# Audio-WestlakeU/NBSS

Measured on AMD Instinct MI355X. Metric: utterances/sec (4 s, 6ch, 129 freqs) SpatialNet bf16 train at 1/2/4/8 MI355X, higher is better.
Workload: dtype bf16; 1 GPU; SpatialNet-small 6ch->2spk, 4-s 8-kHz utterances (32000 samples), n_fft 256/hop 128 (F=129, T=251), 8 layers, full train step (STFT..Adam), bf16 stream + fp32 master/stats, 32 utterances per GPU per step; batch_per_gpu=32, global_batch=32, parallelism=dp1

## Files before the change

nbss_amd/csrc/tconvffn_s.hip:

```cpp
#include "side.h"
#include "launch.h"
#include "layout.h"
#include "prof.h"
#include "fold.h"
#include "foldk.h"

#define TS_H 96
#define TS_FFN 192
#define TS_G 8
#define TS_CG 24
#define TS_RS 200
#define TS_PAD 4
#define TS_ONE 0x3F80u
#define TS_WL_FR 56

typedef float f32x16 __attribute__((ext_vector_type(16)));
typedef Frag<bf16_t> FragH;

NBSS_DEV f32x16 mma32(const FragH& a, const FragH& b, f32x16 c) {
#ifdef NBSS_EMU
    return hipemu::mfma_32x32x16_bf16(a.v, b.v, c);
#else
    return __builtin_amdgcn_mfma_f32_32x32x16_bf16(a.v, b.v, c, 0, 0, 0);
#endif
// ... 774 lines not shown
                        pa.d[i] = pack2bf(a3[2 * i], a3[2 * i + 1]) & vm;
                        const float v0 = bf_lo(pa.d[i]), v1 = bf_hi(pa.d[i]);
                        s1 += v0 + v1;
                        s2 += v0 * v0 + v1 * v1;
                    }
                    p6_store(orow(t, 2, 6), pa);
                }
        }
        s1 = wave_sum64(s1);
        s2 = wave_sum64(s2);
        if (L.lane == 0) {
            red[(gl * 2 + th) * 2] = s1;
            red[(gl * 2 + th) * 2 + 1] = s2;
        }
    }
    load_wfrags<5>(wb, W.C2T, g, L.lane);
    PHASE(6);
    lds_barrier();
    PHASE(7);
    const float gmean = (red[gl * 4] + red[gl * 4 + 2]) / cnt;
    const float grstd = rsqrtf(fmaxf((red[gl * 4 + 1] + red[gl * 4 + 3]) / cnt - gmean * gmean, 0.f) + 1e-5f);
#pragma unroll 2
    for (int s = s_beg; s < s_end; ++s) {
        const int t = 32 * s + L.n;
        const bool tv = t < T_;
        const uint32_t vm = lane_mask(tv);
        bf16_t* r = orow(t, 2, 6);
        P6 pa, pn, ph;
        p6_load(r, pa);
        float a3[12], hv[12];
        p6_unpack(pa, a3);
#pragma unroll
        for (int q = 0; q < 12; ++q) a3[q] = (a3[q] - gmean) * grstd;
        p6_pack(a3, vm, pn);
        p6_unpack(pn, a3);
#pragma unroll
        for (int q = 0; q < 12; ++q) hv[q] = silu_f(a3[q] * gw[q] + gb[q]);
        p6_pack(hv, vm, ph);
        p6_store(Bc + (size_t)t * TB_RS, pn);
        p6_store(r, ph);
    }
    run_gstore(ops.h4, 2, 6);
    PHASE(8);
    lds_barrier();
    PHASE(9);
#pragma unroll 1
    TB_BLOCKS(true) {
        FragH b[TB_SB][5];
        P6 p5[TB_SB];
#pragma unroll
        for (int k = 0; k < TB_SB; ++k)
            if (s0 + k < s_end) {
                const int t = 32 * (s0 + k) + L.n;
                conv_bfrags3(L, rowp(t - 1, 2, 6), rowp(t, 2, 6), rowp(t + 1, 2, 6), b[k]);
                const int pi = s0 + k - s_beg;
#pragma unroll
                for (int i = 0; i < 6; ++i) {
                    const uint32_t lo = pi == 0 ? park0.d[i] : park1.d[i], hi = pi == 2 ? park2.d[i] : park3.d[i];
                    p5[k].d[i] = pi < 2 ? lo : hi;
                }
            }
#pragma unroll
        for (int k = 0; k < TB_SB; ++k)
            if (s0 + k < s_end) {
                const int t = 32 * (s0 + k) + L.n;
                const bool tv = t < T_;
                const uint32_t vm = lane_mask(tv);
                const f32x16 a5 = conv_mma(wc, b[k]);
                float hv[12], dv[12], d5[12];
                p6_unpack(p5[k], d5);
#pragma unroll
                for (int r = 0; r < 12; ++r) {
                    silu_dsilu(a5[r], hv[r], dv[r]);
                    dv[r] *= d5[r];
                }
                P6 ph, pd;
                p6_pack(hv, vm, ph);
                p6_pack(dv, vm, pd);
                p6_store(orow(t, 1, 7), pd);
                p6_gstore(ops.h5 + gbase + (size_t)t * TS_CG, ph, tv, true);
            }
    }
    run_gstore(ops.da5, 1, 7);
    load_wfrags<5>(wc, W.C3T, g, L.lane);
    PHASE(10);
    lds_barrier();
    PHASE(11);
    fetch_cross(1, 7);
    {
        float sa = 0.f, sb = 0.f, dgw[12], dgb[12];
#pragma unroll
        for (int r = 0; r < 12; ++r) dgw[r] = dgb[r] = 0.f;
#pragma unroll 1
        TB_BLOCKS(false) {
            FragH b[TB_SB][5];
#pragma unroll
            for (int k = 0; k < TB_SB; ++k)
                if (s0 + k < s_end) {
                    const int t = 32 * (s0 + k) + L.n;
                    conv_bfrags3(L, rowx(t - 1, 1, 7), rowp(t, 1, 7), rowx(t + 1, 1, 7), b[k]);
                }
#pragma unroll
            for (int k = 0; k < TB_SB; ++k)
                if (s0 + k < s_end) {
                    const int t = 32 * (s0 + k) + L.n;
                    const uint32_t vm = lane_mask(t < T_);
                    const f32x16 dh4 = conv_mma(wc, b[k]);
                    P6 pn, pd;
                    p6_load(Bc + (size_t)t * TB_RS, pn);
                    float ah[12], dn[12];
                    p6_unpack(pn, ah);
#pragma unroll
                    for (int r = 0; r < 12; ++r) dn[r] = dh4[r] * dsilu_only(ah[r] * gw[r] + gb[r]);
                    p6_pack(dn, vm, pd);
                    p6_unpack(pd, dn);
#pragma unroll
                    for (int r = 0; r < 12; ++r) {
                        dgw[r] += dn[r] * ah[r];
                        dgb[r] += dn[r];
                        sa += gw[r] * dn[r];
                        sb += gw[r] * dn[r] * ah[r];
                    }
                    p6_store(orow(t, 2, 6), pd);
                }
        }
        sa = wave_sum64(sa);
        sb = wave_sum64(sb);
        if (L.lane == 0) {
            red[(gl * 2 + th) * 2] = sa;
            red[(gl * 2 + th) * 2 + 1] = sb;
        }
#pragma unroll
        for (int r = 0; r < 12; ++r) {
            const float a = half_sum32(dgw[r]), bq = half_sum32(dgb[r]);
            if (L.n == 0) {
                const int ch = gl * TS_CG + (r & 3) + 8 * (r >> 2) + 4 * L.h;
                gnp[(th * 2 + 0) * 96 + ch] = a;
                gnp[(th * 2 + 1) * 96 + ch] = bq;
            }
        }
        if (L.lane < 6) *reinterpret_cast<u32x2*>(Sc + (size_t)(th ? NT + 6 : 1) * TB_RS + 4 * L.lane) = (u32x2){0u, 0u};
    }
    PHASE(12);
    lds_barrier();
    PHASE(13);
    {
        const float msa = (red[gl * 4] + red[gl * 4 + 2]) / cnt, msb = (red[gl * 4 + 1] + red[gl * 4 + 3]) / cnt;
#pragma unroll 2
        for (int s = s_beg; s < s_end; ++s) {
            const int t = 32 * s + L.n;
            const bool tv = t < T_;
            const uint32_t vm = lane_mask(tv);
            bf16_t* r = orow(t, 2, 6);
            P6 pd, pn, po;
            p6_load(r, pd);
            p6_load(Bc + (size_t)t * TB_RS, pn);
            float dn[12], ah[12];
            p6_unpack(pd, dn);
            p6_unpack(pn, ah);
#pragma unroll
            for (int q = 0; q < 12; ++q) dn[q] = grstd * (gw[q] * dn[q] - msa - ah[q] * msb);
            p6_pack(dn, vm, po);
            p6_store(r, po);
        }
        run_gstore(ops.da3, 2, 6);
    }
    PHASE(14);
    lds_barrier();
    PHASE(15);
    fetch_cross(2, 6);
#pragma unroll 1
    TB_BLOCKS(false) {
        FragH b[TB_SB][5];
#pragma unroll
        for (int k = 0; k < TB_SB; ++k)
            if (s0 + k < s_end) {
                const int t = 32 * (s0 + k) + L.n;
                conv_bfrags3(L, rowx(t - 1, 2, 6), rowp(t, 2, 6), rowx(t + 1, 2, 6), b[k]);
            }
#pragma unroll
        for (int k = 0; k < TB_SB; ++k)
            if (s0 + k < s_end) {
                const int t = 32 * (s0 + k) + L.n;
                const bool tv = t < T_;
                const uint32_t vm = lane_mask(tv);
                const f32x16 dh2 = conv_mma(wb, b[k]);
                P6 pd2, po;
                p6_load(Ac + (size_t)t * TB_RS, pd2);
                float d2[12], o[12];
                p6_unpack(pd2, d2);
#pragma unroll
                for (int r = 0; r < 12; ++r) o[r] = dh2[r] * d2[r];
                p6_pack(o, vm, po);
                p6_store(orow(t, 3, 5), po);
            }
    }
    run_gstore(ops.da2, 3, 5);
    if (L.lane < 6) *reinterpret_cast<u32x2*>(Sc + (size_t)(th ? NT + 5 : 2) * TB_RS + 4 * L.lane) = (u32x2){0u, 0u};
    PHASE(16);
    lds_barrier();
    PHASE(17);
    fetch_cross(3, 5);
#pragma unroll 1
    TB_BLOCKS(false) {
        FragH b[TB_SB][5];
#pragma unroll
        for (int k = 0; k < TB_SB; ++k)
            if (s0 + k < s_end) {
                const int t = 32 * (s0 + k) + L.n;
                conv_bfrags3(L, rowx(t - 1, 3, 5), rowp(t, 3, 5), rowx(t + 1, 3, 5), b[k]);
            }
#pragma unroll
        for (int k = 0; k < TB_SB; ++k)
            if (s0 + k < s_end) {
                const int t = 32 * (s0 + k) + L.n;
                const f32x16 dh1 = conv_mma(wa, b[k]);
                float o[12];
#pragma unroll
                for (int r = 0; r < 12; ++r) o[r] = dh1[r];
                P6 po;
                p6_pack(o, 0xFFFFFFFFu, po);
                p6_store(orow(t, 4, 4), po);
            }
    }
    PHASE(18);
    lds_barrier();
    if (w < NS) {
        const int t = 32 * w + L.n;
        const bool tv = t < T_;
#pragma unroll
        for (int q = 0; q < 4; ++q) {
            P6 ph, po;
            p6_load(S + (size_t)(4 + t) * TB_RS + q * TS_CG + 4 * L.h, ph);
            float dh[12], d1[12];
            p6_unpack(ph, dh);
            p6_unpack(d1keep[q], d1);
#pragma unroll
            for (int r = 0; r < 12; ++r) dh[r] *= d1[r];
            p6_pack(dh, lane_mask(tv), po);
            p6_store(S + (size_t)(4 + t) * TB_RS + q * TS_CG + 4 * L.h, po);
        }
        wave_lds_sync();
#pragma unroll
        for (int q = 0; q < 4; ++q)
            rows_gstore<96>(ops.da1 + ((size_t)(4 * gh + q) * ntok + n0 + 32 * w) * TS_CG, S + (size_t)(4 + 32 * w) * TB_RS + q * TS_CG, 32, T_ - 32 * w);
    }
#undef TB_BLOCKS
    for (int i = tid; i < 2 * 96; i += blockDim.x) {
        const int kind = i / 96, ch = i % 96;
        part[(size_t)row * pstride + kind * TS_FFN + gh * 96 + ch] = gnp[(0 * 2 + kind) * 96 + ch] + gnp[(1 * 2 + kind) * 96 + ch];
    }
    PHASE_END();
}
PHASE_READER(nbss_phase_read_tconvffn_bwd_s)

int tconvffn_bwd_s_launch(const nbss_cfg& c, const LayerPtrs& lp, float* part, const void* packed, int layer, const void* x, const void* dy,
                          void* const* opsv, float* stats, int pstride, hipStream_t st) {
    if (c.dtype != NBSS_BF16 || c.T > 256) return NBSS_EUNSUPPORTED;
    const size_t NT = (size_t)((c.T + 31) / 32) * 32;
    const size_t a_el = NT * TB_RS > (size_t)52 * 512 ? NT * TB_RS : (size_t)52 * 512;
    const size_t lds = ((NT + TB_PAD) * TB_RS + a_el + NT * TB_RS) * sizeof(bf16_t) + (16 + 4 * 96) * sizeof(float) + 8 * TS_CG * sizeof(bf16_t) + PHASE_LDS_BYTES;
    if (lds > 160 * 1024) return NBSS_EUNSUPPORTED;
    const bf16_t* pk = (const bf16_t*)packed;
    TsBwdW W = {pk + pack_off(c, layer, K_TS_W1),  pk + pack_off(c, layer, K_TS_W2_T), pk + pack_off(c, layer, K_TS_C1),  pk + pack_off(c, layer, K_TS_C2),
                pk + pack_off(c, layer, K_TS_C3),  pk + pack_off(c, layer, K_TS_C1_T), pk + pack_off(c, layer, K_TS_C2_T), pk + pack_off(c, layer, K_TS_C3_T)};
    TsOps ops = {(bf16_t*)opsv[0], (bf16_t*)opsv[1], (bf16_t*)opsv[2], (bf16_t*)opsv[3], (bf16_t*)opsv[4], (bf16_t*)opsv[5], (bf16_t*)opsv[6], (bf16_t*)opsv[7]};
    int e = NBSS_SET_MAX_LDS(tconvffn_bwd_s_kernel, lds);
    if (e) return e;
    NBSS_LAUNCH(tconvffn_bwd_s_kernel, dim3(2 * c.B * c.F), dim3(512), lds, st, c, lp, W, (const bf16_t*)x, (const bf16_t*)dy, part, ops, stats, pstride);
    return NBSS_CHECK_LAUNCH();
}

struct TvIn {
    const bf16_t *a1, *a2, *a3;
    const float* gn;
};
struct TvW {
    const bf16_t *W2T, *C1T, *C2T, *C3T, *C3;
};
#define TV_CONVW (TS_FFN * TS_CG * 3)
#define TQ_RS 56
#define TQ_PSTRIDE (5 * TS_FFN)
#define TQ_P16 (3 * TV_CONVW)

template <int RS>
NBSS_DEV void tv_contract_t(const bf16_t* Sg, const bf16_t* Hg, int bl, int bu, int NS, int NSL, int mt, f32x4 (&acc)[5], f32x4& bsum) {
    const int lane = lane_id(), l15 = lane & 15, g4 = lane >> 4;
    const int rowoff = 8 * (g4 >> 1) + (g4 & 1) + 2 * (l15 >> 2);
    int boff[5];
#pragma unroll
    for (int j = 0; j < 5; ++j) {
        int pc = 4 * j + (l15 & 3);
        pc = pc < 18 ? pc : 17;
        const int tap = pc / 6, ch4 = pc - 6 * tap;
        boff[j] = (tap + rowoff) * RS + 4 * ch4;
    }
    const int aoff = rowoff * RS + 16 * mt + 4 * (l15 & 3);
    Frag<bf16_t> ones;
#pragma unroll
    for (int jq = 0; jq < 8; ++jq) frag_set(ones, jq, 1.0f);
#pragma unroll
    for (int j = 0; j < 5; ++j) acc[j] = F32X4_ZERO;
    bsum = F32X4_ZERO;
    for (int ks = 0; ks < NS; ++ks) {
        const int base = (ks < NSL ? bl : bu) + 32 * ks;
        Frag<bf16_t> fa, fb[5];
        frag_load_tr(fa, Sg + (size_t)base * RS + aoff, RS);
#pragma unroll
        for (int j = 0; j < 5; ++j) frag_load_tr(fb[j], Hg + (size_t)(32 * ks) * RS + boff[j], RS);
        bsum = mma(fa, ones, bsum);
#pragma unroll
        for (int j = 0; j < 5; ++j) acc[j] = mma(fa, fb[j], acc[j]);
    }
}
NBSS_DEV void tv_flush(bf16_t* __restrict__ w16, float* __restrict__ brow, int g, int mt, const f32x4 (&acc)[5], const f32x4& bsum) {
    const int lane = lane_id(), l15 = lane & 15, g4 = lane >> 4;
    const int oc0 = 16 * mt + 4 * g4;
    if (oc0 < TS_CG) {
        const int o0 = g * TS_CG + oc0;
#pragma unroll
        for (int j = 0; j < 5; ++j) {
            const int pc = 4 * j + (l15 >> 2);
            if (pc < 18) {
                const int tap = pc / 6, i = (pc - 6 * tap) * 4 + (l15 & 3);
                const u32x2 v = {pack2bf(acc[j][0], acc[j][1]), pack2bf(acc[j][2], acc[j][3])};
                *reinterpret_cast<u32x2*>(w16 + (((size_t)g * 3 + tap) * TS_CG + i) * TS_CG + oc0) = v;
            }
        }
        if (l15 == 0) {
#pragma unroll
            for (int r = 0; r < 4; ++r) brow[o0 + r] = bsum[r];
        }
    }
}

#define TV_RSL 64
static_assert(TS_H == FK_H && TS_FFN == FK_FFN && TS_CG == FK_TCG && TV_CONVW == FK_TCONVW, "foldk.h");
__global__ __launch_bounds__(256) void tconv_part_reduce1_kernel(const bf16_t* __restrict__ part16, int nrows, float* __restrict__ slices, int P16) {
    fk_p16_slices(part16, nrows, slices, P16, (int)blockIdx.x, (int)blockIdx.y, (int)gridDim.y);
}
__global__ __launch_bounds__(256) void tconv_part_reduce2_kernel(const float* __restrict__ slices, int nsl, float* __restrict__ G, long long off0, long long off1, long long off2,
                                                                 long long off3, int P16) {
    fk_tconv_final(slices, nsl, G, off0, off1, off2, off3, P16, (int)blockIdx.x);
}

__global__ __launch_bounds__(256, 2) void tconvffn_bwd_q_kernel(nbss_cfg c, LayerPtrs lp, TvW W, TvIn sv, const bf16_t* __restrict__ dy, float* __restrict__ part,
                                                                bf16_t* __restrict__ part16, bf16_t* __restrict__ op_h5, bf16_t* __restrict__ op_da1, int flip) {
    NBSS_LDS(smem);
    const int T_ = c.T, NS = (T_ + 31) >> 5, NT = NS * 32, NSL = NS >> 1, TS = 32 * NSL;
    bf16_t* S = reinterpret_cast<bf16_t*>(smem);
    bf16_t* H = S + (size_t)(NT + TB_PAD) * TQ_RS;
    const size_t h_el = (size_t)(NT + 2) * TQ_RS > (size_t)12 * 512 ? (size_t)(NT + 2) * TQ_RS : (size_t)12 * 512;
    float* red = reinterpret_cast<float*>(H + h_el);
    float* gnp = red + 8;
    bf16_t* mbox = reinterpret_cast<bf16_t*>(gnp + 4 * 48);
    bf16_t* wl = H;
    PHASE_BEGIN(mbox + 4 * TS_CG);
    const TsLane L;
    const int w = wave_id_u(), tid = threadIdx.x;
    const int row0 = blockIdx.x >> 2, gq = blockIdx.x & 3, row = flip ? (int)(gridDim.x >> 2) - 1 - row0 : row0;
    const size_t n0 = (size_t)row * T_, ntok = (size_t)c.B * c.F * T_;
    const bf16_t* dyb = dy + n0 * TS_H;

    const int gl = w >> 1, th = w & 1, g = 2 * gq + gl;
    const int s_beg = th ? NSL : 0, s_end = th ? NS : NSL, nblk = (s_end - s_beg + TB_SB - 1) / TB_SB;
    const size_t gsv = ((size_t)g * ntok + n0) * TS_CG + 4 * L.h;
    P6 pn0, pn1, pn2, pn3, pd0, pd1, pd2, pd3, ra0, ra1, ra2, ra3;
#define TV_LOADA(k, src, dst)                                                        \
    {                                                                                \
        const int t_ = 32 * (s_beg + (k)) + L.n, tc_ = t_ < T_ ? t_ : T_ - 1;        \
        if (s_beg + (k) < s_end) p6_gload((src) + gsv + (size_t)tc_ * TS_CG, dst);   \
        else                                                                         \
            for (int i_ = 0; i_ < 6; ++i_) dst.d[i_] = 0u;                           \
    }
#define TV_LOADA4(src) TV_LOADA(0, src, ra0) TV_LOADA(1, src, ra1) TV_LOADA(2, src, ra2) TV_LOADA(3, src, ra3)
    {
        u32x4 wr[3];
#pragma unroll
        for (int i = 0; i < 3; ++i) wr[i] = reinterpret_cast<const u32x4*>(W.W2T + (size_t)gq * 12 * 512)[tid + i * 256];
        u32x4 rawd[2][6];
#pragma unroll
        for (int k2 = 0; k2 < 2; ++k2) {
            const int t = 32 * (w + 4 * k2) + L.n, tc = t < T_ ? t : T_ - 1;
#pragma unroll
            for (int ks = 0; ks < 6; ++ks) rawd[k2][ks] = *reinterpret_cast<const u32x4*>(dyb + (size_t)tc * TS_H + 16 * ks + 8 * L.h);
        }
        TV_LOADA4(sv.a3)
        for (int i = tid; i < 4 * TQ_RS / 2; i += 256) reinterpret_cast<uint32_t*>(S)[i] = 0u;
        for (int i = tid; i < 5 * TQ_RS / 2; i += 256) reinterpret_cast<uint32_t*>(S + (size_t)(NT + 4) * TQ_RS)[i] = 0u;
#pragma unroll
        for (int i = 0; i < 3; ++i) reinterpret_cast<u32x4*>(wl)[tid + i * 256] = wr[i];
        PHASE(0);
        lds_barrier();
        PHASE(1);
#pragma unroll
        for (int k2 = 0; k2 < 2; ++k2) {
            const int sw = w + 4 * k2, t = 32 * sw + L.n;
            if (sw < NS) {
                const uint32_t vm = lane_mask(t < T_);
                FragH dq[6];
#pragma unroll
                for (int ks = 0; ks < 6; ++ks) dq[ks].v = __builtin_bit_cast(s16x8, rawd[k2][ks]);
                bf16_t* srow = S + (size_t)((sw < NSL ? 1 : 7) + t) * TQ_RS + 4 * L.h;
#pragma unroll
                for (int q = 0; q < 2; ++q) {
                    FragH w2t[6];
                    load_wfrags<6>(w2t, wl, q, L.lane);
                    f32x16 d5 = mma32(w2t[0], dq[0], f32x16_zero());
#pragma unroll
                    for (int ks = 1; ks < 6; ++ks) d5 = mma32(w2t[ks], dq[ks], d5);
                    float dv[12];
#pragma unroll
                    for (int r = 0; r < 12; ++r) dv[r] = d5[r];
                    P6 pd;
                    p6_pack(dv, vm, pd);
                    p6_store(srow + q * TS_CG, pd);
                }
            }
        }
    }
    PHASE(2);

    bf16_t* Sc = S + gl * TS_CG;
    bf16_t* Hc = H + gl * TS_CG;
    const int run0 = 32 * s_beg, nrun = 32 * (s_end - s_beg);
    auto rowp = [&](int tt, int bl, int bu) -> const bf16_t* { return Sc + (size_t)((tt < TS ? bl : bu) + tt) * TQ_RS; };
    auto orow = [&](int tt, int bl, int bu) -> bf16_t* { return Sc + (size_t)((th ? bu : bl) + tt) * TQ_RS + 4 * L.h; };
    bf16_t* mb = mbox + w * TS_CG;
    auto fetch_cross = [&](int bl, int bu) {
        const bf16_t* src = Sc + (size_t)(th ? bl + TS - 1 : bu + TS) * TQ_RS;
        if (L.lane < 6) *reinterpret_cast<u32x2*>(mb + 4 * L.lane) = *reinterpret_cast<const u32x2*>(src + 4 * L.lane);
        lds_barrier();
    };
    auto rowx = [&](int tt, int bl, int bu) -> const bf16_t* {
        const bool lower = tt < TS;
        const bf16_t* r = Sc + (size_t)((lower ? bl : bu) + tt) * TQ_RS;
        return lower != (th == 0) ? mb : r;
    };
    float gw[12], gb[12];
    chan_vec12(lp.p[P_TF_GN_W] + g * TS_CG, L.h, gw);
    chan_vec12(lp.p[P_TF_GN_B] + g * TS_CG, L.h, gb);
    const float cnt = (float)(TS_CG * T_);
    const float gmean = sv.gn[((size_t)row * TS_G + g) * 2], grstd = sv.gn[((size_t)row * TS_G + g) * 2 + 1];
    float* prow = part + (size_t)row * TQ_PSTRIDE + 2 * TS_FFN;
    bf16_t* prow16 = part16 + (size_t)row * TQ_P16;

    FragH wt[5];
    load_wfrags<5>(wt, W.C3T, g, L.lane);
#define TV_PICK(dst, k_, hib_, q0, q1, q2, q3)                                                            \
    for (int i_ = 0; i_ < 6; ++i_) {                                                                      \
        const uint32_t lo_ = (k_) == 0 ? q0.d[i_] : q1.d[i_], hi_ = (k_) == 0 ? q2.d[i_] : q3.d[i_];      \
        dst.d[i_] = (hib_) ? hi_ : lo_;                                                                   \
    }
#define TB_BLOCKS(fwd_dir)                                                   \
    for (int bi_ = 0; bi_ < nblk; ++bi_)                                     \
        for (int s0 = s_beg + TB_SB * (((fwd_dir) == (th == 0)) ? bi_ : nblk - 1 - bi_), once_ = 1; once_; once_ = 0)

    lds_barrier();
    PHASE(3);
    if (L.lane < 6) *reinterpret_cast<u32x2*>(Hc + (size_t)(th ? NT + 1 : 0) * TQ_RS + 4 * L.lane) = (u32x2){0u, 0u};
#define TV_STAGE1(k, RA, PN, PD)                                                          \
    if (s_beg + (k) < s_end) {                                                            \
        const int t = 32 * (s_beg + (k)) + L.n;                                           \
        const uint32_t vm = lane_mask(t < T_);                                            \
        float a3[12], hv[12], dv[12];                                                     \
        p6_unpack(RA, a3);                                                                \
        for (int q = 0; q < 12; ++q) a3[q] = (a3[q] - gmean) * grstd;                     \
        p6_pack(a3, vm, PN);                                                              \
        p6_unpack(PN, a3);                                                                \
        for (int q = 0; q < 12; ++q) silu_dsilu(a3[q] * gw[q] + gb[q], hv[q], dv[q]);     \
        P6 ph;                                                                            \
        p6_pack(hv, vm, ph);                                                              \
        p6_pack(dv, vm, PD);                                                              \
        p6_store(Hc + (size_t)(1 + t) * TQ_RS + 4 * L.h, ph);                             \
    } else {                                                                              \
        for (int i_ = 0; i_ < 6; ++i_) PN.d[i_] = PD.d[i_] = 0u;                          \
    }
    TV_STAGE1(0, ra0, pn0, pd0)
    TV_STAGE1(1, ra1, pn1, pd1)
    TV_STAGE1(2, ra2, pn2, pd2)
    TV_STAGE1(3, ra3, pn3, pd3)
#undef TV_STAGE1
    TV_LOADA4(sv.a2)
    PHASE(4);
    lds_barrier();
    {
        FragH wf[5];
        load_wfrags<5>(wf, W.C3, g, L.lane);
#pragma unroll 1
        for (int s0 = s_beg; s0 < s_end; s0 += TB_SB) {
            FragH b[TB_SB][5];
#pragma unroll
            for (int k = 0; k < TB_SB; ++k)
                if (s0 + k < s_end) {
                    const bf16_t* r1 = Hc + (size_t)(1 + 32 * (s0 + k) + L.n) * TQ_RS;
                    conv_bfrags3(L, r1 - TQ_RS, r1, r1 + TQ_RS, b[k]);
                }
#pragma unroll
            for (int k = 0; k < TB_SB; ++k)
                if (s0 + k < s_end) {
                    const int t = 32 * (s0 + k) + L.n;
                    const bool tv = t < T_;
                    const uint32_t vm = lane_mask(tv);
                    const f32x16 a5 = conv_mma(wf, b[k]);
                    bf16_t* r = orow(t, 1, 7);
                    P6 p5, ph, pd;
                    p6_load(r, p5);
                    float hv[12], dv[12], d5[12];
                    p6_unpack(p5, d5);
#pragma unroll
                    for (int q = 0; q < 12; ++q) {
                        silu_dsilu(a5[q], hv[q], dv[q]);
                        dv[q] *= d5[q];
                    }
                    p6_pack(hv, vm, ph);
                    p6_pack(dv, vm, pd);
                    p6_store(r, pd);
                    p6_gstore(op_h5 + gsv + (size_t)t * TS_CG, ph, tv, true);
                }
        }
    }
    lds_barrier();
    PHASE(5);
    {
        f32x4 acc[5], bsum;
        tv_contract_t<TQ_RS>(Sc, Hc, 1, 7, NS, NSL, th, acc, bsum);
        tv_flush(prow16 + 2 * TV_CONVW, prow + 2 * TS_FFN, g, th, acc, bsum);
    }
    PHASE(6);
    fetch_cross(1, 7);
    PHASE(7);
    {
        float sa = 0.f, sb = 0.f, dgw[12], dgb[12];
#pragma unroll
        for (int r = 0; r < 12; ++r) dgw[r] = dgb[r] = 0.f;
#pragma unroll 1
        TB_BLOCKS(false) {
            FragH b[TB_SB][5];
            const bool hib = s0 - s_beg >= 2;
#pragma unroll
            for (int k = 0; k < TB_SB; ++k)
                if (s0 + k < s_end) {
                    const int t = 32 * (s0 + k) + L.n;
                    conv_bfrags3(L, rowx(t - 1, 1, 7), rowp(t, 1, 7), rowx(t + 1, 1, 7), b[k]);
                }
#pragma unroll
            for (int k = 0; k < TB_SB; ++k)
                if (s0 + k < s_end) {
                    const int t = 32 * (s0 + k) + L.n;
                    const uint32_t vm = lane_mask(t < T_);
                    const f32x16 dh4 = conv_mma(wt, b[k]);
                    P6 pn, pdv, pd;
                    TV_PICK(pn, k, hib, pn0, pn1, pn2, pn3)
                    TV_PICK(pdv, k, hib, pd0, pd1, pd2, pd3)
                    float ah[12], d4[12], dn[12];
                    p6_unpack(pn, ah);
                    p6_unpack(pdv, d4);
#pragma unroll
                    for (int r = 0; r < 12; ++r) dn[r] = dh4[r] * d4[r];
                    p6_pack(dn, vm, pd);
                    p6_unpack(pd, dn);
#pragma unroll
                    for (int r = 0; r < 12; ++r) {
                        dgw[r] += dn[r] * ah[r];
                        dgb[r] += dn[r];
                        sa += gw[r] * dn[r];
                        sb += gw[r] * dn[r] * ah[r];
                    }
                    p6_store(orow(t, 2, 6), pd);
                }
        }
        sa = wave_sum64(sa);
        sb = wave_sum64(sb);
        if (L.lane == 0) {
            red[(gl * 2 + th) * 2] = sa;
            red[(gl * 2 + th) * 2 + 1] = sb;
        }
#pragma unroll
        for (int r = 0; r < 12; ++r) {
            const float a = half_sum32(dgw[r]), bq = half_sum32(dgb[r]);
            if (L.n == 0) {
                const int ch = gl * TS_CG + (r & 3) + 8 * (r >> 2) + 4 * L.h;
                gnp[(th * 2 + 0) * 48 + ch] = a;
                gnp[(th * 2 + 1) * 48 + ch] = bq;
            }
        }
        if (L.lane < 6) *reinterpret_cast<u32x2*>(Sc + (size_t)(th ? NT + 6 : 1) * TQ_RS + 4 * L.lane) = (u32x2){0u, 0u};
    }
    load_wfrags<5>(wt, W.C2T, g, L.lane);
    PHASE(8);
    lds_barrier();
    PHASE(9);
    {
        const float msa = (red[gl * 4] + red[gl * 4 + 2]) / cnt, msb = (red[gl * 4 + 1] + red[gl * 4 + 3]) / cnt;
#define TV_STAGE3B(k, RA, PN, PD)                                                         \
    if (s_beg + (k) < s_end) {                                                            \
        const int t = 32 * (s_beg + (k)) + L.n;                                           \
        const uint32_t vm = lane_mask(t < T_);                                            \
        bf16_t* r = orow(t, 2, 6);                                                        \
        P6 pdn, po, ph;                                                                   \
        p6_load(r, pdn);                                                                  \
        float dn[12], ah[12], a2[12], hv[12], dv[12];                                     \
        p6_unpack(pdn, dn);                                                               \
        p6_unpack(PN, ah);                                                                \
        for (int q = 0; q < 12; ++q) dn[q] = grstd * (gw[q] * dn[q] - msa - ah[q] * msb); \
        p6_pack(dn, vm, po);                                                              \
        p6_store(r, po);                                                                  \
        p6_unpack(RA, a2);                                                                \
        for (int q = 0; q < 12; ++q) silu_dsilu(a2[q], hv[q], dv[q]);                     \
        p6_pack(hv, vm, ph);                                                              \
        p6_pack(dv, vm, PD);                                                              \
        p6_store(Hc + (size_t)(1 + t) * TQ_RS + 4 * L.h, ph);                             \
    }
        TV_STAGE3B(0, ra0, pn0, pd0)
        TV_STAGE3B(1, ra1, pn1, pd1)
        TV_STAGE3B(2, ra2, pn2, pd2)
        TV_STAGE3B(3, ra3, pn3, pd3)
#undef TV_STAGE3B
        TV_LOADA4(sv.a1)
    }
    PHASE(10);
    lds_barrier();
    PHASE(11);
    {
        f32x4 acc[5], bsum;
        tv_contract_t<TQ_RS>(Sc, Hc, 2, 6, NS, NSL, th, acc, bsum);
        tv_flush(prow16 + 1 * TV_CONVW, prow + 1 * TS_FFN, g, th, acc, bsum);
    }
    PHASE(12);
    fetch_cross(2, 6);
    PHASE(13);
#pragma unroll 1
    TB_BLOCKS(false) {
        FragH b[TB_SB][5];
        const bool hib = s0 - s_beg >= 2;
#pragma unroll
        for (int k = 0; k < TB_SB; ++k)
            if (s0 + k < s_end) {
                const int t = 32 * (s0 + k) + L.n;
                conv_bfrags3(L, rowx(t - 1, 2, 6), rowp(t, 2, 6), rowx(t + 1, 2, 6), b[k]);
            }
#pragma unroll
        for (int k = 0; k < TB_SB; ++k)
            if (s0 + k < s_end) {
                const int t = 32 * (s0 + k) + L.n;
                const uint32_t vm = lane_mask(t < T_);
                const f32x16 dh2 = conv_mma(wt, b[k]);
                P6 pdv, po;
                TV_PICK(pdv, k, hib, pd0, pd1, pd2, pd3)
                float d2[12], o[12];
                p6_unpack(pdv, d2);
#pragma unroll
                for (int r = 0; r < 12; ++r) o[r] = dh2[r] * d2[r];
                p6_pack(o, vm, po);
                p6_store(orow(t, 3, 5), po);
            }
    }
    if (L.lane < 6) *reinterpret_cast<u32x2*>(Sc + (size_t)(th ? NT + 5 : 2) * TQ_RS + 4 * L.lane) = (u32x2){0u, 0u};
    load_wfrags<5>(wt, W.C1T, g, L.lane);
#define TV_STAGE5(k, RA, PN)                                                              \
    if (s_beg + (k) < s_end) {                                                            \
        const int t = 32 * (s_beg + (k)) + L.n;                                           \
        const uint32_t vm = lane_mask(t < T_);                                            \
        float a1[12], hv[12], dv[12];                                                     \
        P6 ph;                                                                            \
        p6_unpack(RA, a1);                                                                \
        for (int q = 0; q < 12; ++q) silu_dsilu(a1[q], hv[q], dv[q]);                     \
        p6_pack(hv, vm, ph);                                                              \
        p6_pack(dv, vm, PN);                                                              \
        p6_store(Hc + (size_t)(1 + t) * TQ_RS + 4 * L.h, ph);                             \
    }
    TV_STAGE5(0, ra0, pn0)
    TV_STAGE5(1, ra1, pn1)
    TV_STAGE5(2, ra2, pn2)
    TV_STAGE5(3, ra3, pn3)
#undef TV_STAGE5
    PHASE(14);
    lds_barrier();
    PHASE(15);
    {
        f32x4 acc[5], bsum;
        tv_contract_t<TQ_RS>(Sc, Hc, 3, 5, NS, NSL, th, acc, bsum);
        tv_flush(prow16, prow, g, th, acc, bsum);
    }
    PHASE(16);
    fetch_cross(3, 5);
    PHASE(17);
#pragma unroll 1
    TB_BLOCKS(false) {
        FragH b[TB_SB][5];
        const bool hib = s0 - s_beg >= 2;
#pragma unroll
        for (int k = 0; k < TB_SB; ++k)
            if (s0 + k < s_end) {
                const int t = 32 * (s0 + k) + L.n;
                conv_bfrags3(L, rowx(t - 1, 3, 5), rowp(t, 3, 5), rowx(t + 1, 3, 5), b[k]);
            }
#pragma unroll
        for (int k = 0; k < TB_SB; ++k)
            if (s0 + k < s_end) {
                const int t = 32 * (s0 + k) + L.n;
                const uint32_t vm = lane_mask(t < T_);
                const f32x16 dh1 = conv_mma(wt, b[k]);
                P6 pdv, po;
                TV_PICK(pdv, k, hib, pn0, pn1, pn2, pn3)
                float d1[12], o[12];
                p6_unpack(pdv, d1);
#pragma unroll
                for (int r = 0; r < 12; ++r) o[r] = dh1[r] * d1[r];
                p6_pack(o, vm, po);
                p6_store(orow(t, 4, 4), po);
            }
    }
    wave_lds_sync();
    rows_gstore_t<128 * 3, TQ_RS>(op_da1 + ((size_t)g * ntok + n0 + run0) * TS_CG, Sc + (size_t)(4 + run0) * TQ_RS, nrun, T_ - run0);
    PHASE(18);
#undef TB_BLOCKS
#undef TV_PICK
#undef TV_LOADA4
#undef TV_LOADA
    for (int i = tid; i < 2 * 48; i += 256) {
        const int kind = i / 48, ch = i % 48;
        part[(size_t)row * TQ_PSTRIDE + kind * TS_FFN + gq * 48 + ch] = gnp[(0 * 2 + kind) * 48 + ch] + gnp[(1 * 2 + kind) * 48 + ch];
    }
    PHASE_END();
}

int part16_slices_launch(const void* part16, int nrows, float* slices, int p16, int* nsl_out, hipStream_t st, bool batch) {
    const int nsl = nrows < TV_RSL ? nrows : TV_RSL;
    *nsl_out = nsl;
    if (g_fold && batch) {
        g_fold->st = st;
        FoldItem it;
        it.kind = FK_P16_SLICES;
        it.gx = (p16 / 8 + 255) / 256; it.gy = nsl; it.nblk = it.gx * it.gy;
        it.u.p16.part16 = part16; it.u.p16.nrows = nrows; it.u.p16.p16 = p16; it.u.p16.nsl = nsl; it.u.p16.slices = slices; it.u.p16.G = nullptr;
        return g_fold->add(1, it);
    }
    NBSS_FOLD_LAUNCH(tconv_part_reduce1_kernel, dim3((p16 / 8 + 255) / 256, nsl), dim3(256), 0, st, (const bf16_t*)part16, nrows, slices, p16);
    return NBSS_CHECK_LAUNCH();
}
int tconvffn_v_reduce16(const nbss_cfg& c, const void* part16, float* slices, float* G, const long long* offs, hipStream_t st) {
    const int nrows = c.B * c.F, nsl = nrows < TV_RSL ? nrows : TV_RSL, p16 = TQ_P16;
    if (g_fold) {
        int err;
        void* sl = g_fold->alloc((size_t)nsl * p16 * sizeof(float), &err);
        if (err) return err;
        if (sl) {
            g_fold->st = st;
            FoldItem it;
            it.kind = FK_P16_SLICES;
            it.gx = (p16 / 8 + 255) / 256; it.gy = nsl; it.nblk = it.gx * it.gy;
            it.u.p16.part16 = part16; it.u.p16.nrows = nrows; it.u.p16.p16 = p16; it.u.p16.nsl = nsl; it.u.p16.slices = (float*)sl; it.u.p16.G = G;
            for (int k = 0; k < 3; ++k) it.u.p16.off[k] = offs[k];
            it.u.p16.off[3] = 0;
            if ((err = g_fold->add(1, it))) return err;
            it.kind = FK_TCONV_FINAL;
            it.gx = (p16 + 255) / 256; it.gy = 1; it.nblk = it.gx;
            return g_fold->add(2, it);
        }
        if ((err = g_fold->flush())) return err;
    }
    NBSS_FOLD_LAUNCH(tconv_part_reduce1_kernel, dim3((p16 / 8 + 255) / 256, nsl), dim3(256), 0, st, (const bf16_t*)part16, nrows, slices, p16);
    int e = NBSS_CHECK_LAUNCH();
    if (e) return e;
    NBSS_FOLD_LAUNCH(tconv_part_reduce2_kernel, dim3((p16 + 255) / 256), dim3(256), 0, st, (const float*)slices, nsl, G, offs[0], offs[1], offs[2], 0LL, p16);
    return NBSS_CHECK_LAUNCH();
}
int tconvffn_bwd_q_launch(const nbss_cfg& c, const LayerPtrs& lp, float* part, const void* packed, int layer, const void* dy, void* tsave, void* op_h5, void* op_da1,
                          hipStream_t st) {
    bf16_t* part16 = reinterpret_cast<bf16_t*>(part + (size_t)c.B * c.F * TQ_PSTRIDE);
    if (c.dtype != NBSS_BF16 || c.T > 256 || !tsave) return NBSS_EUNSUPPORTED;
    const size_t NT = (size_t)((c.T + 31) / 32) * 32;
    const size_t h_el = (NT + 2) * TQ_RS > (size_t)12 * 512 ? (NT + 2) * TQ_RS : (size_t)12 * 512;
    const size_t lds = ((NT + TB_PAD) * TQ_RS + h_el) * sizeof(bf16_t) + (8 + 4 * 48) * sizeof(float) + 4 * TS_CG * sizeof(bf16_t) + PHASE_LDS_BYTES;
    const bf16_t* pk = (const bf16_t*)packed;
    TvW W = {pk + pack_off(c, layer, K_TS_W2_T), pk + pack_off(c, layer, K_TS_C1_T), pk + pack_off(c, layer, K_TS_C2_T), pk + pack_off(c, layer, K_TS_C3_T),
             pk + pack_off(c, layer, K_TS_C3)};
    const TsSave s = ts_save_ptrs(c, tsave);
    TvIn in = {s.a1, s.a2, s.a3, s.gn};
    int e = NBSS_SET_MAX_LDS(tconvffn_bwd_q_kernel, lds);
    if (e) return e;
    NBSS_LAUNCH(tconvffn_bwd_q_kernel, dim3(4 * c.B * c.F), dim3(256), lds, st, c, lp, W, in, (const bf16_t*)dy, part, part16, (bf16_t*)op_h5, (bf16_t*)op_da1,
                walk_flip_next());
    return NBSS_CHECK_LAUNCH();
}
float* tconvffn_save_ln_stats(const nbss_cfg& c, void* tsave) { return ts_save_ptrs(c, tsave).ln; }
```

Measured before the change: 736.9 utterances/s.

## Specialize T-conv FFN backward kernel for eight 32-step time slabs

Adds a template variant of the temporal-conv FFN backward kernel for T in (224,256], which fixes NS=8. The slab count, masks and edge-row selection become compile-time, most bounds checks drop away, and the block loops can be unrolled. It also inserts sched_barrier fences and empty-asm register parking to constrain scheduling and register pressure. Global pointer arithmetic is split into a size_t base plus a 32-bit offset. The specialization is selected by default for T=251 and can be disabled with an environment variable, at the cost of more code to maintain and a new risk of masking bugs.

```diff
diff --git a/nbss_amd/csrc/tconvffn_s.hip b/nbss_amd/csrc/tconvffn_s.hip
--- a/nbss_amd/csrc/tconvffn_s.hip
+++ b/nbss_amd/csrc/tconvffn_s.hip
@@ -1100,6 +1100,7 @@
 #pragma unroll
     for (int j = 0; j < 5; ++j) acc[j] = F32X4_ZERO;
     bsum = F32X4_ZERO;
+#pragma unroll 1
     for (int ks = 0; ks < NS; ++ks) {
         const int base = (ks < NSL ? bl : bu) + 32 * ks;
         Frag<bf16_t> fa, fb[5];
@@ -1142,10 +1143,24 @@
     fk_tconv_final(slices, nsl, G, off0, off1, off2, off3, P16, (int)blockIdx.x);
 }
 
+NBSS_DEV void tv_fence(bool on) {
+#ifndef NBSS_EMU
+    if (on) __builtin_amdgcn_sched_barrier(0);
+#endif
+}
+NBSS_DEV void tv_park(bool on, P6& p) {
+#ifndef NBSS_EMU
+    if (on) {
+#pragma unroll
+        for (int i = 0; i < 6; ++i) asm volatile("" : "+v"(p.d[i]));
+    }
+#endif
+}
+template <bool T8>
 __global__ __launch_bounds__(256, 2) void tconvffn_bwd_q_kernel(nbss_cfg c, LayerPtrs lp, TvW W, TvIn sv, const bf16_t* __restrict__ dy, float* __restrict__ part,
                                                                 bf16_t* __restrict__ part16, bf16_t* __restrict__ op_h5, bf16_t* __restrict__ op_da1, int flip) {
     NBSS_LDS(smem);
-    const int T_ = c.T, NS = (T_ + 31) >> 5, NT = NS * 32, NSL = NS >> 1, TS = 32 * NSL;
+    const int T_ = c.T, NS = T8 ? 8 : (T_ + 31) >> 5, NT = NS * 32, NSL = NS >> 1, TS = 32 * NSL;
     bf16_t* S = reinterpret_cast<bf16_t*>(smem);
     bf16_t* H = S + (size_t)(NT + TB_PAD) * TQ_RS;
     const size_t h_el = (size_t)(NT + 2) * TQ_RS > (size_t)12 * 512 ? (size_t)(NT + 2) * TQ_RS : (size_t)12 * 512;
@@ -1162,14 +1177,19 @@
 
     const int gl = w >> 1, th = w & 1, g = 2 * gq + gl;
     const int s_beg = th ? NSL : 0, s_end = th ? NS : NSL, nblk = (s_end - s_beg + TB_SB - 1) / TB_SB;
-    const size_t gsv = ((size_t)g * ntok + n0) * TS_CG + 4 * L.h;
+    const size_t gsu = ((size_t)g * ntok + n0) * TS_CG;
+#define TV_GPTR(base, s, tc) ((base) + (gsu + (size_t)(s) * (32 * TS_CG)) + (uint32_t)(((tc)-32 * (s)) * TS_CG + 4 * L.h))
+    const int sx = T8 && th == 0 ? 2 : 0;
+    const uint32_t vm3 = lane_mask(th == 0 || 224 + L.n < T_);
+#define TV_SLOT_T(k) (32 * (s_beg + ((k) ^ sx)) + L.n)
+#define TV_SLOT_VM(k, t) (T8 ? ((k) == 3 ? vm3 : 0xFFFFFFFFu) : lane_mask((t) < T_))
     P6 pn0, pn1, pn2, pn3, pd0, pd1, pd2, pd3, ra0, ra1, ra2, ra3;
-#define TV_LOADA(k, src, dst)                                                        \
-    {                                                                                \
-        const int t_ = 32 * (s_beg + (k)) + L.n, tc_ = t_ < T_ ? t_ : T_ - 1;        \
-        if (s_beg + (k) < s_end) p6_gload((src) + gsv + (size_t)tc_ * TS_CG, dst);   \
-        else                                                                         \
-            for (int i_ = 0; i_ < 6; ++i_) dst.d[i_] = 0u;                           \
+#define TV_LOADA(k, src, dst)                                                                    \
+    {                                                                                            \
+        const int t_ = TV_SLOT_T(k), tc_ = (T8 && (k) != 3) || t_ < T_ ? t_ : T_ - 1;            \
+        if (T8 || s_beg + (k) < s_end) p6_gload(TV_GPTR(src, s_beg + ((k) ^ sx), tc_), dst);     \
+        else                                                                                     \
+            for (int i_ = 0; i_ < 6; ++i_) dst.d[i_] = 0u;                                       \
     }
 #define TV_LOADA4(src) TV_LOADA(0, src, ra0) TV_LOADA(1, src, ra1) TV_LOADA(2, src, ra2) TV_LOADA(3, src, ra3)
     {
@@ -1179,7 +1199,7 @@
         u32x4 rawd[2][6];
 #pragma unroll
         for (int k2 = 0; k2 < 2; ++k2) {
-            const int t = 32 * (w + 4 * k2) + L.n, tc = t < T_ ? t : T_ - 1;
+            const int t = 32 * (w + 4 * k2) + L.n, tc = (T8 && k2 == 0) || t < T_ ? t : T_ - 1;
 #pragma unroll
             for (int ks = 0; ks < 6; ++ks) rawd[k2][ks] = *reinterpret_cast<const u32x4*>(dyb + (size_t)tc * TS_H + 16 * ks + 8 * L.h);
         }
@@ -1194,12 +1214,12 @@
 #pragma unroll
         for (int k2 = 0; k2 < 2; ++k2) {
             const int sw = w + 4 * k2, t = 32 * sw + L.n;
-            if (sw < NS) {
-                const uint32_t vm = lane_mask(t < T_);
+            if (T8 || sw < NS) {
+                const uint32_t vm = T8 && k2 == 0 ? 0xFFFFFFFFu : lane_mask(t < T_);
                 FragH dq[6];
 #pragma unroll
                 for (int ks = 0; ks < 6; ++ks) dq[ks].v = __builtin_bit_cast(s16x8, rawd[k2][ks]);
-                bf16_t* srow = S + (size_t)((sw < NSL ? 1 : 7) + t) * TQ_RS + 4 * L.h;
+                bf16_t* srow = S + (size_t)(((T8 ? k2 == 0 : sw < NSL) ? 1 : 7) + t) * TQ_RS + 4 * L.h;
 #pragma unroll
                 for (int q = 0; q < 2; ++q) {
                     FragH w2t[6];
@@ -1214,6 +1234,7 @@
                     p6_pack(dv, vm, pd);
                     p6_store(srow + q * TS_CG, pd);
                 }
+                tv_fence(T8);
             }
         }
     }
@@ -1222,7 +1243,7 @@
     bf16_t* Sc = S + gl * TS_CG;
     bf16_t* Hc = H + gl * TS_CG;
     const int run0 = 32 * s_beg, nrun = 32 * (s_end - s_beg);
-    auto rowp = [&](int tt, int bl, int bu) -> const bf16_t* { return Sc + (size_t)((tt < TS ? bl : bu) + tt) * TQ_RS; };
+    auto rowp = [&](int tt, int bl, int bu) -> const bf16_t* { return Sc + (size_t)((th ? bu : bl) + tt) * TQ_RS; };
     auto orow = [&](int tt, int bl, int bu) -> bf16_t* { return Sc + (size_t)((th ? bu : bl) + tt) * TQ_RS + 4 * L.h; };
     bf16_t* mb = mbox + w * TS_CG;
     auto fetch_cross = [&](int bl, int bu) {
@@ -1230,10 +1251,9 @@
         if (L.lane < 6) *reinterpret_cast<u32x2*>(mb + 4 * L.lane) = *reinterpret_cast<const u32x2*>(src + 4 * L.lane);
         lds_barrier();
     };
-    auto rowx = [&](int tt, int bl, int bu) -> const bf16_t* {
-        const bool lower = tt < TS;
-        const bf16_t* r = Sc + (size_t)((lower ? bl : bu) + tt) * TQ_RS;
-        return lower != (th == 0) ? mb : r;
+    auto rowx = [&](int tt, int bl, int bu, bool edge) -> const bf16_t* {
+        const bf16_t* r = Sc + (size_t)((th ? bu : bl) + tt) * TQ_RS;
+        return edge && tt == (th ? TS - 1 : TS) ? mb : r;
     };
     float gw[12], gb[12];
     chan_vec12(lp.p[P_TF_GN_W] + g * TS_CG, L.h, gw);
@@ -1250,17 +1270,20 @@
         const uint32_t lo_ = (k_) == 0 ? q0.d[i_] : q1.d[i_], hi_ = (k_) == 0 ? q2.d[i_] : q3.d[i_];      \
         dst.d[i_] = (hib_) ? hi_ : lo_;                                                                   \
     }
-#define TB_BLOCKS(fwd_dir)                                                   \
-    for (int bi_ = 0; bi_ < nblk; ++bi_)                                     \
-        for (int s0 = s_beg + TB_SB * (((fwd_dir) == (th == 0)) ? bi_ : nblk - 1 - bi_), once_ = 1; once_; once_ = 0)
+    constexpr int TV_UB = T8 ? 2 : 1;
+#define TB_BLOCKS                                                                                                           \
+    for (int bi_ = 0; bi_ < (T8 ? 2 : nblk); ++bi_)                                                                         \
+        for (int s0 = s_beg + TB_SB * (T8 ? bi_ ^ (sx >> 1) : th ? bi_ : nblk - 1 - bi_), once_ = 1; once_; once_ = 0)
+#define TB_HIB (T8 ? bi_ == 1 : s0 - s_beg >= 2)
+#define TB_SLOT(k) (T8 ? 2 * bi_ + (k) : s0 - s_beg + (k))
 
     lds_barrier();
     PHASE(3);
     if (L.lane < 6) *reinterpret_cast<u32x2*>(Hc + (size_t)(th ? NT + 1 : 0) * TQ_RS + 4 * L.lane) = (u32x2){0u, 0u};
 #define TV_STAGE1(k, RA, PN, PD)                                                          \
-    if (s_beg + (k) < s_end) {                                                            \
-        const int t = 32 * (s_beg + (k)) + L.n;                                           \
-        const uint32_t vm = lane_mask(t < T_);                                            \
+    if (T8 || s_beg + (k) < s_end) {                                                      \
+        const int t = TV_SLOT_T(k);                                                       \
+        const uint32_t vm = TV_SLOT_VM(k, t);                                             \
         float a3[12], hv[12], dv[12];                                                     \
         p6_unpack(RA, a3);                                                                \
         for (int q = 0; q < 12; ++q) a3[q] = (a3[q] - gmean) * grstd;                     \
@@ -1271,6 +1294,9 @@
         p6_pack(hv, vm, ph);                                                              \
         p6_pack(dv, vm, PD);                                                              \
         p6_store(Hc + (size_t)(1 + t) * TQ_RS + 4 * L.h, ph);                             \
+        tv_park(T8, PN);                                                                  \
+        tv_park(T8, PD);                                                                  \
+        tv_fence(T8);                                                                     \
     } else {                                                                              \
         for (int i_ = 0; i_ < 6; ++i_) PN.d[i_] = PD.d[i_] = 0u;                          \
     }
@@ -1286,20 +1312,21 @@
         FragH wf[5];
         load_wfrags<5>(wf, W.C3, g, L.lane);
 #pragma unroll 1
-        for (int s0 = s_beg; s0 < s_end; s0 += TB_SB) {
+        for (int bi_ = 0; bi_ < (T8 ? 2 : nblk); ++bi_) {
+            const int s0 = s_beg + TB_SB * bi_;
             FragH b[TB_SB][5];
 #pragma unroll
             for (int k = 0; k < TB_SB; ++k)
-                if (s0 + k < s_end) {
+                if (T8 || s0 + k < s_end) {
                     const bf16_t* r1 = Hc + (size_t)(1 + 32 * (s0 + k) + L.n) * TQ_RS;
                     conv_bfrags3(L, r1 - TQ_RS, r1, r1 + TQ_RS, b[k]);
                 }
 #pragma unroll
             for (int k = 0; k < TB_SB; ++k)
-                if (s0 + k < s_end) {
+                if (T8 || s0 + k < s_end) {
                     const int t = 32 * (s0 + k) + L.n;
-                    const bool tv = t < T_;
-                    const uint32_t vm = lane_mask(tv);
+                    const bool tv = (T8 && 2 * bi_ + k != 3) || t < T_;
+                    const uint32_t vm = TV_SLOT_VM(2 * bi_ + k, t);
                     const f32x16 a5 = conv_mma(wf, b[k]);
                     bf16_t* r = orow(t, 1, 7);
                     P6 p5, ph, pd;
@@ -1314,7 +1341,7 @@
                     p6_pack(hv, vm, ph);
                     p6_pack(dv, vm, pd);
                     p6_store(r, pd);
-                    p6_gstore(op_h5 + gsv + (size_t)t * TS_CG, ph, tv, true);
+                    p6_gstore(TV_GPTR(op_h5, s0 + k, t), ph, tv, true);
                 }
         }
     }
@@ -1332,21 +1359,21 @@
         float sa = 0.f, sb = 0.f, dgw[12], dgb[12];
 #pragma unroll
         for (int r = 0; r < 12; ++r) dgw[r] = dgb[r] = 0.f;
-#pragma unroll 1
-        TB_BLOCKS(false) {
+#pragma unroll TV_UB
+        TB_BLOCKS {
             FragH b[TB_SB][5];
-            const bool hib = s0 - s_beg >= 2;
+            const bool hib = TB_HIB;
 #pragma unroll
             for (int k = 0; k < TB_SB; ++k)
-                if (s0 + k < s_end) {
+                if (T8 || s0 + k < s_end) {
                     const int t = 32 * (s0 + k) + L.n;
-                    conv_bfrags3(L, rowx(t - 1, 1, 7), rowp(t, 1, 7), rowx(t + 1, 1, 7), b[k]);
+                    conv_bfrags3(L, rowx(t - 1, 1, 7, !T8 || TB_SLOT(k) == 0), rowp(t, 1, 7), rowx(t + 1, 1, 7, !T8 || TB_SLOT(k) == 1), b[k]);
                 }
 #pragma unroll
             for (int k = 0; k < TB_SB; ++k)
-                if (s0 + k < s_end) {
+                if (T8 || s0 + k < s_end) {
                     const int t = 32 * (s0 + k) + L.n;
-                    const uint32_t vm = lane_mask(t < T_);
+                    const uint32_t vm = TV_SLOT_VM(TB_SLOT(k), t);
                     const f32x16 dh4 = conv_mma(wt, b[k]);
                     P6 pn, pdv, pd;
                     TV_PICK(pn, k, hib, pn0, pn1, pn2, pn3)
@@ -1366,6 +1393,7 @@
                         sb += gw[r] * dn[r] * ah[r];
                     }
                     p6_store(orow(t, 2, 6), pd);
+                    tv_fence(T8);
                 }
         }
         sa = wave_sum64(sa);
@@ -1392,9 +1420,9 @@
     {
         const float msa = (red[gl * 4] + red[gl * 4 + 2]) / cnt, msb = (red[gl * 4 + 1] + red[gl * 4 + 3]) / cnt;
 #define TV_STAGE3B(k, RA, PN, PD)                                                         \
-    if (s_beg + (k) < s_end) {                                                            \
-        const int t = 32 * (s_beg + (k)) + L.n;                                           \
-        const uint32_t vm = lane_mask(t < T_);                                            \
+    if (T8 || s_beg + (k) < s_end) {                                                      \
+        const int t = TV_SLOT_T(k);                                                       \
+        const uint32_t vm = TV_SLOT_VM(k, t);                                             \
         bf16_t* r = orow(t, 2, 6);                                                        \
         P6 pdn, po, ph;                                                                   \
         p6_load(r, pdn);                                                                  \
@@ -1409,6 +1437,8 @@
         p6_pack(hv, vm, ph);                                                              \
         p6_pack(dv, vm, PD);                                                              \
         p6_store(Hc + (size_t)(1 + t) * TQ_RS + 4 * L.h, ph);                             \
+        tv_park(T8, PD);                                                                  \
+        tv_fence(T8);                                                                     \
     }
         TV_STAGE3B(0, ra0, pn0, pd0)
         TV_STAGE3B(1, ra1, pn1, pd1)
@@ -1428,21 +1458,21 @@
     PHASE(12);
     fetch_cross(2, 6);
     PHASE(13);
-#pragma unroll 1
-    TB_BLOCKS(false) {
+#pragma unroll TV_UB
+    TB_BLOCKS {
         FragH b[TB_SB][5];
-        const bool hib = s0 - s_beg >= 2;
+        const bool hib = TB_HIB;
 #pragma unroll
         for (int k = 0; k < TB_SB; ++k)
-            if (s0 + k < s_end) {
+            if (T8 || s0 + k < s_end) {
                 const int t = 32 * (s0 + k) + L.n;
-                conv_bfrags3(L, rowx(t - 1, 2, 6), rowp(t, 2, 6), rowx(t + 1, 2, 6), b[k]);
+                conv_bfrags3(L, rowx(t - 1, 2, 6, !T8 || TB_SLOT(k) == 0), rowp(t, 2, 6), rowx(t + 1, 2, 6, !T8 || TB_SLOT(k) == 1), b[k]);
             }
 #pragma unroll
         for (int k = 0; k < TB_SB; ++k)
-            if (s0 + k < s_end) {
+            if (T8 || s0 + k < s_end) {
                 const int t = 32 * (s0 + k) + L.n;
-                const uint32_t vm = lane_mask(t < T_);
+                const uint32_t vm = TV_SLOT_VM(TB_SLOT(k), t);
                 const f32x16 dh2 = conv_mma(wt, b[k]);
                 P6 pdv, po;
                 TV_PICK(pdv, k, hib, pd0, pd1, pd2, pd3)
@@ -1452,14 +1482,15 @@
                 for (int r = 0; r < 12; ++r) o[r] = dh2[r] * d2[r];
                 p6_pack(o, vm, po);
                 p6_store(orow(t, 3, 5), po);
+                    tv_fence(T8);
             }
     }
     if (L.lane < 6) *reinterpret_cast<u32x2*>(Sc + (size_t)(th ? NT + 5 : 2) * TQ_RS + 4 * L.lane) = (u32x2){0u, 0u};
     load_wfrags<5>(wt, W.C1T, g, L.lane);
 #define TV_STAGE5(k, RA, PN)                                                              \
-    if (s_beg + (k) < s_end) {                                                            \
-        const int t = 32 * (s_beg + (k)) + L.n;                                           \
-        const uint32_t vm = lane_mask(t < T_);                                            \
+    if (T8 || s_beg + (k) < s_end) {                                                      \
+        const int t = TV_SLOT_T(k);                                                       \
+        const uint32_t vm = TV_SLOT_VM(k, t);                                             \
         float a1[12], hv[12], dv[12];                                                     \
         P6 ph;                                                                            \
         p6_unpack(RA, a1);                                                                \
@@ -1467,6 +1498,8 @@
         p6_pack(hv, vm, ph);                                                              \
         p6_pack(dv, vm, PN);                                                              \
         p6_store(Hc + (size_t)(1 + t) * TQ_RS + 4 * L.h, ph);                             \
+        tv_park(T8, PN);                                                                  \
+        tv_fence(T8);                                                                     \
     }
     TV_STAGE5(0, ra0, pn0)
     TV_STAGE5(1, ra1, pn1)
@@ -1484,21 +1517,21 @@
     PHASE(16);
     fetch_cross(3, 5);
     PHASE(17);
-#pragma unroll 1
-    TB_BLOCKS(false) {
+#pragma unroll TV_UB
+    TB_BLOCKS {
         FragH b[TB_SB][5];
-        const bool hib = s0 - s_beg >= 2;
+        const bool hib = TB_HIB;
 #pragma unroll
         for (int k = 0; k < TB_SB; ++k)
-            if (s0 + k < s_end) {
+            if (T8 || s0 + k < s_end) {
                 const int t = 32 * (s0 + k) + L.n;
-                conv_bfrags3(L, rowx(t - 1, 3, 5), rowp(t, 3, 5), rowx(t + 1, 3, 5), b[k]);
+                conv_bfrags3(L, rowx(t - 1, 3, 5, !T8 || TB_SLOT(k) == 0), rowp(t, 3, 5), rowx(t + 1, 3, 5, !T8 || TB_SLOT(k) == 1), b[k]);
             }
 #pragma unroll
         for (int k = 0; k < TB_SB; ++k)
-            if (s0 + k < s_end) {
+            if (T8 || s0 + k < s_end) {
                 const int t = 32 * (s0 + k) + L.n;
-                const uint32_t vm = lane_mask(t < T_);
+                const uint32_t vm = TV_SLOT_VM(TB_SLOT(k), t);
                 const f32x16 dh1 = conv_mma(wt, b[k]);
                 P6 pdv, po;
                 TV_PICK(pdv, k, hib, pn0, pn1, pn2, pn3)
@@ -1508,12 +1541,18 @@
                 for (int r = 0; r < 12; ++r) o[r] = dh1[r] * d1[r];
                 p6_pack(o, vm, po);
                 p6_store(orow(t, 4, 4), po);
+                    tv_fence(T8);
             }
     }
     wave_lds_sync();
     rows_gstore_t<128 * 3, TQ_RS>(op_da1 + ((size_t)g * ntok + n0 + run0) * TS_CG, Sc + (size_t)(4 + run0) * TQ_RS, nrun, T_ - run0);
     PHASE(18);
+#undef TB_SLOT
+#undef TB_HIB
 #undef TB_BLOCKS
+#undef TV_GPTR
+#undef TV_SLOT_VM
+#undef TV_SLOT_T
 #undef TV_PICK
 #undef TV_LOADA4
 #undef TV_LOADA
@@ -1577,10 +1616,18 @@
              pk + pack_off(c, layer, K_TS_C3)};
     const TsSave s = ts_save_ptrs(c, tsave);
     TvIn in = {s.a1, s.a2, s.a3, s.gn};
-    int e = NBSS_SET_MAX_LDS(tconvffn_bwd_q_kernel, lds);
-    if (e) return e;
-    NBSS_LAUNCH(tconvffn_bwd_q_kernel, dim3(4 * c.B * c.F), dim3(256), lds, st, c, lp, W, in, (const bf16_t*)dy, part, part16, (bf16_t*)op_h5, (bf16_t*)op_da1,
-                walk_flip_next());
+    static const bool t8_off = [] { const char* v = getenv("NBSS_TCF_T8"); return v && v[0] == '0'; }();
+    const int flip = walk_flip_next();
+    int e;
+    if (c.T > 224 && !t8_off) {
+        if ((e = NBSS_SET_MAX_LDS(tconvffn_bwd_q_kernel<true>, lds))) return e;
+        NBSS_LAUNCH(tconvffn_bwd_q_kernel<true>, dim3(4 * c.B * c.F), dim3(256), lds, st, c, lp, W, in, (const bf16_t*)dy, part, part16, (bf16_t*)op_h5,
+                    (bf16_t*)op_da1, flip);
+    } else {
+        if ((e = NBSS_SET_MAX_LDS(tconvffn_bwd_q_kernel<false>, lds))) return e;
+        NBSS_LAUNCH(tconvffn_bwd_q_kernel<false>, dim3(4 * c.B * c.F), dim3(256), lds, st, c, lp, W, in, (const bf16_t*)dy, part, part16, (bf16_t*)op_h5,
+                    (bf16_t*)op_da1, flip);
+    }
     return NBSS_CHECK_LAUNCH();
 }
 float* tconvffn_save_ln_stats(const nbss_cfg& c, void* tsave) { return ts_save_ptrs(c, tsave).ln; }
```

Result: slower. 726.5 utterances/s (-1.4%).
